# PaddlePaddle/Parakeet

Measured on AMD Instinct MI355X. Metric: audio samples/sec, FastSpeech2+PWGAN 22.05kHz, higher is better.
Workload: dtype f32 (3-term split-fp16 MFMA, fp32-equivalent; exact-fp32 in roofline.exact_f32); 1 GPU; FastSpeech2+PWG end-to-end (BASELINE config 4 per-GPU share): 32 utterances/GPU x 128 phonemes -> 640 frames -> 163840 samples each, LJSpeech architecture, random-init weights; utterances_per_gpu=32, global_batch=32, minibatch=32, parallelism=dp1 (utterance sharding, no data-path collective)

## Files before the change

parakeet_amd/csrc/pwg.hip:

```cpp
#include <cmath>
#include <cstdlib>

#include "pk_gemm.h"
#include "pk_split.h"
#include "pwg_gen.h"

typedef float f32x16 __attribute__((ext_vector_type(16)));
typedef float f32x4 __attribute__((ext_vector_type(4)));
typedef float f32x2 __attribute__((ext_vector_type(2)));
#ifndef PK_PWG_TILE_MAP
#define PK_PWG_TILE_MAP 1
#endif
#ifndef PK_PWG_NT_SKIP
#define PK_PWG_NT_SKIP 1
#endif
#ifndef PK_PWG_SKIP_SCOPE
#define PK_PWG_SKIP_SCOPE 0
#endif
#ifndef PK_PWG_NT_EDGE
#define PK_PWG_NT_EDGE 0
#endif
#ifndef PK_PWG_AMAX_PROBE
#define PK_PWG_AMAX_PROBE 0
#endif
#ifndef PK_PWG_NT_XOUT
#define PK_PWG_NT_XOUT 1
#endif
#ifndef PK_PWG_SKIP_VEC
#define PK_PWG_SKIP_VEC 1
#endif
#if PK_PWG_SKIP_VEC && PK_PWG_SKIP_SCOPE != 0
#error "PK_PWG_SKIP_SCOPE measures the dword skip stream: build it with PK_PWG_SKIP_VEC=0"
#endif
namespace {
__device__ __forceinline__ f32x4 pwg_skip_ld4(const float* p) {
#if PK_PWG_NT_SKIP
    return __builtin_nontemporal_load(reinterpret_cast<const f32x4*>(p));
#else
    return *reinterpret_cast<const f32x4*>(p);
#endif
}
__device__ __forceinline__ void pwg_skip_st4(f32x4 v, float* p) {
#if PK_PWG_NT_SKIP
    __builtin_nontemporal_store(v, reinterpret_cast<f32x4*>(p));
#else
    *reinterpret_cast<f32x4*>(p) = v;
#endif
}
__device__ __forceinline__ float pwg_skip_ld(const float* p) {
#if PK_PWG_SKIP_SCOPE == 1
    return __hip_atomic_load(p, __ATOMIC_RELAXED, __HIP_MEMORY_SCOPE_AGENT);
#elif PK_PWG_SKIP_SCOPE == 2
    return __hip_atomic_load(p, __ATOMIC_RELAXED, __HIP_MEMORY_SCOPE_SYSTEM);
#elif PK_PWG_SKIP_SCOPE == 3
    return __hip_atomic_load(p, __ATOMIC_RELAXED, __HIP_MEMORY_SCOPE_WORKGROUP);
#elif PK_PWG_NT_SKIP
    return __builtin_nontemporal_load(p);
#else
    return *p;
#endif
}
__device__ __forceinline__ void pwg_skip_st(float v, float* p) {
// ... 245 lines not shown
    float acc = 0.f;
    for (int jj = 0; jj < UPW; ++jj) acc = fmaf(w[jj], P[(long)(row0 + f + jj - 2) * ldp + col0 + co], acc);
    out[(long)co * n_frames * hop + (long)f * hop + phase] = acc;
}

struct PwgLayerArgs {
    const float* xin;
    float* xout;
    float* skip;
    const float* w1;
    const float* w2;
    const float* bias;
    const float* P;
    const float* uptab;
    const int* tile_t0;
    const int* tile_cls;
    long Ttot;
    int ldp;
    int ntiles;
    int dilation;
    int dbg;
    const unsigned* xe_in;
    unsigned* xe_out;
    int k1;
    float i0, i1;
    const int* tile_kx_in;
    const int* tile_kx_out;
    const float* noise;
    const float* nz_tab;
    float nz_wmax, nz_bmax;
    long noise_n;
    unsigned* amax_out;
    PwgGen gen;
};

__device__ __forceinline__ float gated(float a, float b) {
    a = __builtin_amdgcn_fmed3f(a, -10.f, 10.f);
    const float ea = __expf(-2.f * a);
    const float eb = __expf(-b);
    return (1.f - ea) * __builtin_amdgcn_rcpf((1.f + ea) * (1.f + eb));
}

constexpr float PK_Z_SCALE = PK_UNIT_SCALE;
template <int CTRL, int ROW_MASK>
__device__ __forceinline__ float dpp_max_step(float v) {
    const int t = __builtin_amdgcn_update_dpp(__float_as_int(v), __float_as_int(v), CTRL, ROW_MASK, 0xf, false);
    return fmaxf(v, __int_as_float(t));
}
__device__ __forceinline__ float wave_max64(float v) {
    v = dpp_max_step<0xB1, 0xf>(v);
    v = dpp_max_step<0x4E, 0xf>(v);
    v = dpp_max_step<0x124, 0xf>(v);
    v = dpp_max_step<0x128, 0xf>(v);
    v = dpp_max_step<0x142, 0xa>(v);
    v = dpp_max_step<0x143, 0xc>(v);
    return __int_as_float(__builtin_amdgcn_readlane(__float_as_int(v), 63));
}
__device__ __forceinline__ float gated_s(float a, float b, float ca, float cb) {
    const float ta = __builtin_amdgcn_fmed3f(a * ca, -28.853900817779268f, 28.853900817779268f);
    const float ea = __builtin_amdgcn_exp2f(ta);
    const float eb = __builtin_amdgcn_exp2f(b * cb);
    return fmaf(ea, -PK_Z_SCALE, PK_Z_SCALE) * __builtin_amdgcn_rcpf((1.f + ea) * (1.f + eb));
}

__device__ __forceinline__ f32x2 gated_s2(f32x2 a, f32x2 b, float ca, float cb) {
    f32x2 ta = a * ca, tb = b * cb;
// ... 278 lines not shown
}
typedef __fp16 pkh2 __attribute__((ext_vector_type(2)));
template <>
__device__ __forceinline__ void split_x8<f16x8, _Float16, true>(const float (&v)[8], f16x8& hi, f16x8& lo) {
#pragma unroll
    for (int p = 0; p < 4; ++p) {
        const pkh2 h = __builtin_amdgcn_cvt_pkrtz(v[2 * p], v[2 * p + 1]);
        const unsigned hu = __builtin_bit_cast(unsigned, h);
        float l0, l1;
        asm("v_fma_mix_f32 %0, %1, -1.0, %2 op_sel:[0,0,0] op_sel_hi:[1,0,0]" : "=v"(l0) : "v"(hu), "v"(v[2 * p]));
        asm("v_fma_mix_f32 %0, %1, -1.0, %2 op_sel:[1,0,0] op_sel_hi:[1,0,0]" : "=v"(l1) : "v"(hu), "v"(v[2 * p + 1]));
        hi[2 * p] = (_Float16)h[0];
        hi[2 * p + 1] = (_Float16)h[1];
        lo[2 * p] = (_Float16)l0;
        lo[2 * p + 1] = (_Float16)l1;
    }
}

__device__ __forceinline__ void split_x8s(const float (&v)[8], float s, f16x8& hi, f16x8& lo) {
    float t[8];
#pragma unroll
    for (int p = 0; p < 4; ++p) {
        f32x2 u = {v[2 * p], v[2 * p + 1]};
        u *= s;
        t[2 * p] = u[0];
        t[2 * p + 1] = u[1];
    }
    split_x8<f16x8, _Float16, true>(t, hi, lo);
}

template <bool FIRST, bool HALF, int ABL = 0, bool GEN = false, bool PL = false, bool AMAX = false, bool NZ = false>
__global__ __launch_bounds__(LAYER_WAVES * 64, LAYER_WAVES / 4) void k_pwg_layer_b3(PwgLayerArgs a) {
    static_assert(!NZ || (FIRST && PL && !GEN), "noise-fed: the first block of the planes path at hop 256");
    static_assert(!PL || (HALF && ABL == 0), "planes: the block-scaled split-fp16 path only");
    typedef typename Split16<HALF>::vec bf16x8;
    typedef typename Split16<HALF>::elem elem16;
    __shared__ __attribute__((aligned(16))) float lds[GEN ? LDS_TOTAL_GEN : LDS_TOTAL];
    float* lds_bias = lds + LDS_W1 + LDS_W2;
    {
        const f32x4* src = reinterpret_cast<const f32x4*>(NZ ? a.nz_tab : a.w1);
        f32x4* dst = reinterpret_cast<f32x4*>(lds);
        for (int i = threadIdx.x; i < (NZ ? (2048 + 128) * 4 : B3_W1_BYTES) / 16; i += LAYER_WAVES * 64) dst[i] = src[i];
        const f32x4* src2 = reinterpret_cast<const f32x4*>(a.w2);
        f32x4* dst2 = reinterpret_cast<f32x4*>(lds + LDS_W1);
        for (int i = threadIdx.x; i < B3_W2_BYTES / 16; i += LAYER_WAVES * 64) dst2[i] = src2[i];
        if (threadIdx.x < LDS_BIAS) lds_bias[threadIdx.x] = a.bias[threadIdx.x];
    }
    __syncthreads();

    const int lane = threadIdx.x & 63;
    const int wave = threadIdx.x >> 6;
    const int j = lane & 31;
    const int hi = lane >> 5;
    const int d = a.dilation;
    const bf16x8* lds_a = reinterpret_cast<const bf16x8*>(lds) + lane;
    const bf16x8* lds_a2 = reinterpret_cast<const bf16x8*>(lds + LDS_W1) + lane;
    float* lds_p = lds + LDS_W1 + LDS_W2 + LDS_BIAS + wave * (GEN ? LDS_PW_GEN : LDS_PW);

    const int per_xcd = gridDim.x >> 3;
    const int wg_slot = (gridDim.x & 7) == 0 ? (int)(blockIdx.x & 7) * per_xcd + (int)(blockIdx.x >> 3)
                                             : (int)blockIdx.x;
    int my_slot = wg_slot * LAYER_WAVES + wave;
#if PK_PWG_TILE_MAP
    static_assert(LAYER_WAVES == 8, "the tile maps below split a workgroup into waves 0..3 / 4..7 (wave >> 2, wave & 3) and the window into 8 per workgroup");
    if ((gridDim.x & 7) == 0) {
        const int wgl = (int)(blockIdx.x >> 3), win = per_xcd * LAYER_WAVES;
        const int local = PK_PWG_TILE_MAP == 1 ? (wave >> 2) * (win >> 1) + wgl * 4 + (wave & 3)
                        : PK_PWG_TILE_MAP == 2 ? wave * per_xcd + wgl
                                               : (wave & 3) * (win >> 2) + wgl * 2 + (wave >> 2);
        my_slot = (int)(blockIdx.x & 7) * win + local;
    }
#endif
    const int stride_slots = (int)gridDim.x * LAYER_WAVES;
    const int n_wtiles = a.ntiles * (TILE / WAVE_T);

    int eoff = 0;
    if (HALF) {
        const int dc = (d + 31) >> 5, df = d >> 5;
        eoff = lane == 0 ? -dc : (lane == 1 ? -df : (lane == 3 ? df : (lane == 4 ? dc : 0)));
    }
    auto load_amax = [&](int t0, int wt) -> unsigned {
        const long tt0 = (long)(t0 & ~255) + (wt & 7) * WAVE_T;
        return (ABL & 1) ? 0x3f800000u : a.xe_in[(tt0 >> 5) + eoff];
    };
    auto tile_scale_exp = [&](unsigned ev) -> int {
        unsigned m = (unsigned)__builtin_amdgcn_readlane((int)ev, 0);
        const unsigned m1 = (unsigned)__builtin_amdgcn_readlane((int)ev, 1);
        const unsigned m2 = (unsigned)__builtin_amdgcn_readlane((int)ev, 2);
        const unsigned m3 = (unsigned)__builtin_amdgcn_readlane((int)ev, 3);
        const unsigned m4 = (unsigned)__builtin_amdgcn_readlane((int)ev, 4);
        m = m > m1 ? m : m1;
        m = m > m2 ? m : m2;
        m = m > m3 ? m : m3;
        m = m > m4 ? m : m4;
        return blk_scale_exp(m);
    };
    int kx = 0, kx_next = 0;
    float xs_cur = 0.f;
    int kxn_v = 0;

    auto group_row = [&](int g, int e) -> long {
        const int cg = g / 3;
        return (long)(32 * (cg >> 1) + mfma_row(8 * (cg & 1) + e, 0));
    };
    auto lane_off = [&](int t0, int wt, int tap) -> unsigned {
        const long tt = (long)(t0 & ~255) + (wt & 7) * WAVE_T + j + (long)(tap - 1) * d;
        return (unsigned)(xoff(tt) + 4 * hi * XBLK);
// ... 39 lines not shown
            const PwgGenCoord gc = gen_coord(a.gen, tile, wt & 7, j);
            prow = a.gen.P0 + (long)(gc.row0 + gc.fa - 2) * a.ldp;
            wsel = (long)gc.cls * a.gen.hop + gc.phase;
            df_n = gc.df;
            valid_n = gc.valid;
        } else {
            prow = a.P + (long)(tile - 2) * a.ldp;
        }
#pragma unroll
        for (int it = 0; it < 3; ++it) {
            const int idx = lane + 64 * it;
            const int jj = idx >> 5, c4 = idx & 31;
            if (idx < (UPW + (GEN ? 1 : 0)) * (G / 4)) preg[it] = *reinterpret_cast<const f32x4*>(prow + (long)jj * a.ldp + 4 * c4);
        }
        if constexpr (!GEN) wsel = (long)cls * TILE + phase;
        const float* wrow = a.uptab + wsel * UPW_PAD;
        const f32x4 w0 = *reinterpret_cast<const f32x4*>(wrow);
        uw[0] = w0[0]; uw[1] = w0[1]; uw[2] = w0[2]; uw[3] = w0[3];
        uw[4] = wrow[4];
    };
    float nzn[3] = {0.f, 0.f, 0.f};
    int cls_cur = 0;
    auto nz_load = [&](int wt_) {
        const long i0 = (long)wt_ * WAVE_T + j;
#pragma unroll
        for (int k = 0; k < 3; ++k) {
            long i = i0 + k - 1;
            i = i < 0 ? 0 : (i >= a.noise_n ? a.noise_n - 1 : i);
            nzn[k] = a.noise[i];
        }
    };
    unsigned vo8n[3] = {0, 0, 0};
    unsigned pvo8n[3] = {0, 0, 0};
    if (my_slot < n_wtiles) {
        const int t0c = a.tile_t0[my_slot >> 3];
#pragma unroll
        for (int tp = 0; tp < 3; ++tp) {
            vo8n[tp] = lane_off(t0c, my_slot, tp);
            if constexpr (PL) pvo8n[tp] = lane_off_pl(t0c, my_slot, tp);
        }
        prefetch_head(my_slot, __builtin_amdgcn_readfirstlane(t0c & 255));
        if constexpr (NZ) {
            cls_cur = __builtin_amdgcn_readfirstlane(t0c & 255);
            kx = __builtin_amdgcn_readfirstlane(a.tile_kx_in[my_slot >> 3]);
            nz_load(my_slot);
        }
#pragma unroll
        for (int g = 0; g < (NZ ? 0 : B3_RING); ++g) load_group(ring[g], g, vo8n[g % 3], pvo8n[g % 3]);
        if constexpr (NZ) {
        } else if constexpr (PL) {
            kx = __builtin_amdgcn_readfirstlane(a.tile_kx_in[my_slot >> 3]);
            planes_operand(ring[0], ph, pl);
        } else if constexpr (HALF) {
            kx = tile_scale_exp(load_amax(t0c, my_slot));
            if constexpr ((ABL & 2) != 0) {
                ph = __builtin_bit_cast(bf16x8, f32x4{ring[0][0], ring[0][1], ring[0][2], ring[0][3]});
                pl = __builtin_bit_cast(bf16x8, f32x4{ring[0][4], ring[0][5], ring[0][6], ring[0][7]});
            } else
            split_x8s(ring[0], pow2f(kx), ph, pl);
        } else {
            split_x8<bf16x8, elem16, HALF>(ring[0], ph, pl);
        }
    }
    bf16x8 c_ah, c_al;
    if constexpr (!NZ) {
        c_ah = lds_a[0];
        c_al = lds_a[4 * 64];
    }

    int amax_utt = -1;
    unsigned amax_run = 0u;
    for (int wt = my_slot; wt < n_wtiles; wt += stride_slots) {
        const int next_wt = wt + stride_slots < n_wtiles ? wt + stride_slots : wt;
        unsigned vo8[3], pvo8[3];
#pragma unroll
        for (int tp = 0; tp < 3; ++tp) {
            vo8[tp] = vo8n[tp];
            pvo8[tp] = pvo8n[tp];
        }
        const int t0n = a.tile_t0[next_wt >> 3];
        int ko_v = 0;
        int utt_v = 0;
        if constexpr (PL) {
            kxn_v = a.tile_kx_in[next_wt >> 3];
            ko_v = a.tile_kx_out[wt >> 3];
            if constexpr (AMAX) utt_v = a.gen.tile_utt[wt >> 3];
            xs_cur = __uint_as_float(0x3f3504f3u - ((unsigned)kx << 23));
        }
        int cls_next = 0;
        const unsigned vo4 = vo8[1];
#if PK_PWG_SKIP_VEC
        const unsigned svo = (vo4 & ~(unsigned)(XBLK_FLOATS - 1)) + (unsigned)(128 * hi + 4 * j);
#endif
        float x_old[32];
        float nz_cur[3] = {0.f, 0.f, 0.f};
        if constexpr (NZ) {
#pragma unroll
            for (int k = 0; k < 3; ++k) nz_cur[k] = nzn[k];
            nz_load(next_wt);
        }
#pragma unroll
        for (int it = 0; it < 3; ++it) {
            const int idx = lane + 64 * it;
            if (idx < (UPW + (GEN ? 1 : 0)) * (G / 4)) reinterpret_cast<f32x4*>(lds_p)[idx] = preg[it];
        }
        const bool lane_valid = valid_n;
// ... 294 lines not shown
                        if (u != amax_utt) {
                            if (amax_utt >= 0 && lane == 0 && !PK_PWG_AMAX_PROBE)
                                atomicMax(a.amax_out + amax_utt * PWG_AMAX_PARTS + (int)(blockIdx.x & (PWG_AMAX_PARTS - 1)), amax_run);
                            amax_utt = u;
                            amax_run = m;
                        } else {
                            amax_run = amax_run > m ? amax_run : m;
                        }
                    }
                    if constexpr (PL) {
                        const float so = pow2f(__builtin_amdgcn_readfirstlane(ko_v));
                        char* pd = reinterpret_cast<char*>(a.xout) + pvo8[1];
#pragma unroll
                        for (int cg = 0; cg < 4; ++cg) {
                            float t8[8];
#pragma unroll
                            for (int e = 0; e < 8; ++e) t8[e] = acc2[cg >> 1][8 * (cg & 1) + e];
                            pl_f16x8 oh, ol;
                            split_x8s(t8, so, oh, ol);
                            if (PK_PWG_NT_XOUT) {
                                __builtin_nontemporal_store(oh, reinterpret_cast<pl_f16x8*>(pd + cg * 2048));
                                __builtin_nontemporal_store(ol, reinterpret_cast<pl_f16x8*>(pd + cg * 2048 + 16));
                            } else {
                                *reinterpret_cast<pl_f16x8*>(pd + cg * 2048) = oh;
                                *reinterpret_cast<pl_f16x8*>(pd + cg * 2048 + 16) = ol;
                            }
                        }
                    }
                }
            }
        }
        kx = kx_next;
        if constexpr (NZ) cls_cur = cls_next;
    }
    if constexpr (PL && AMAX) {
        if (amax_utt >= 0 && lane == 0 && !PK_PWG_AMAX_PROBE)
            atomicMax(a.amax_out + amax_utt * PWG_AMAX_PARTS + (int)(blockIdx.x & (PWG_AMAX_PARTS - 1)), amax_run);
    }
}

struct PwgLastArgs {
    const float* skip;
    const float* w1;
    const float* b1;
    const float* w2;
    float b2;
    float scale;
    const int* tile_t0;
    long Ttot;
    float* wav;
    int kw;
    PwgGen gen;
};
template <bool GEN>
__device__ __forceinline__ long last_out_index(const PwgLastArgs& a, int tile, int off, bool& valid) {
    if constexpr (GEN) {
        const int b = a.gen.tile_utt[tile];
        const int sidx = a.gen.tile_s0[tile] + off;
        valid = sidx < a.gen.utt_S[b];
        return (long)a.gen.utt_off[b] + sidx;
    } else {
        valid = true;
        return (long)tile * TILE + off;
    }
}

template <bool GEN>
__global__ __launch_bounds__(512) void k_pwg_last(PwgLastArgs a) {
    const int lane = threadIdx.x & 63;
    const int wave = threadIdx.x >> 6;
// ... 118 lines not shown
    bool finalized = false;
    int hop = 256;
    int max_dilation = 512;
    int gap = 512;
    bool use_norm = false;
    std::vector<float> h_mu, h_sigma;
    pk_dbuf d_first_w, d_first_b, d_convin_wT, d_uptab, d_mu, d_sigma;
    pk_dbuf d_w1, d_w2, d_bias;
    pk_dbuf d_w1b, d_w2b, d_w1h, d_w2h;
    int math = PK_PWG_MATH_F16X3;
    pk_dbuf d_waux;
    pk_dbuf d_l1, d_l1b, d_l2, d_l1h;
    float l2_bias = 0.f;
    std::vector<int> k1, k2o, k2s;
    int kw_last = 0;
    pk_dbuf d_bias_h, ws_xe0, ws_xe1;
    pk_dbuf ws_mel, ws_noise, ws_wav, ws_c0, ws_cin, ws_P, ws_x0, ws_x1, ws_skip, ws_dbg;
    pk_dbuf ws_tab;
    std::vector<int> last_frames, last_toff, last_cuL, last_cuC;
    float first_wmax = 0.f, first_bmax = 0.f;
    std::vector<float> first_w_host, first_b_host;
    pk_dbuf d_nz;
    int nz_k1 = 0;
    bool noise_fed = true;
    pk_dbuf d_cl, ws_nmax, ws_tkx;
    int last_ntiles = 0;
    long last_Ttot = 0;
    int last_x_final = 0;
    int last_ldp = 0;
    size_t last_o_cls = 0;
    int dbg = 0;
    bool planes_on = true;
    bool last_planes = false;
    bool last_skip_vec = false;
    int scale_guard = 1;
    bool guard_done = false;
    int guard_every = 16;
    int calls_since_sample = 0;
    int samples_dropped = 0;
    bool sample_pending = false;
    hipEvent_t ev_sample = nullptr;
    float* host_sample = nullptr;
    size_t host_sample_cap = 0;
    int sample_B = 0;
    std::vector<int> sample_frames;
    int deferred_fallbacks = 0;
    bool fell_back = false;
    std::vector<float> overshoot_log2;
    std::vector<float> cl_host;
    pk_dbuf ws_amax;
    unsigned long long seed = 0, rng_offset = 0;
    long chunk_samples = 1L << 40;
    bool generic_shape = false;
    bool generic_opt = false;
    bool gen_active = false;
    pwg_gen* gen = nullptr;
};

template <bool PROF>
static int pwg_ablation_launch(pk_ctx* ctx, int dbg, int grid, dim3 blk, const PwgLayerArgs& a) {
    if constexpr (PROF) {
        if (dbg == 1) PK_LAUNCH(ctx, "pwg_layer_h3", (k_pwg_layer_b3<false, true, 1>), dim3(grid), blk, 0, a);
        else if (dbg == 32) PK_LAUNCH(ctx, "pwg_layer_h3", (k_pwg_layer_b3<false, true, 2>), dim3(grid), blk, 0, a);
        else if (dbg == 96) PK_LAUNCH(ctx, "pwg_layer_h3", (k_pwg_layer_b3<false, true, 6>), dim3(grid), blk, 0, a);
        else if (dbg == 160) PK_LAUNCH(ctx, "pwg_layer_h3", (k_pwg_layer_b3<false, true, 10>), dim3(grid), blk, 0, a);
        else PK_LAUNCH(ctx, "pwg_layer_h3", (k_pwg_layer_b3<false, true>), dim3(grid), blk, 0, a);
        return PK_OK;
    } else {
        PK_FAIL(PK_ESTATE, "ablation switches exist in the profile build only");
    }
}

extern "C" int pk_pwg_create(pk_ctx* ctx, const pk_pwg_cfg* cfg, pk_pwg** out) {
    if (!ctx || !cfg || !out) PK_FAIL(PK_EINVAL, "pk_pwg_create: NULL argument");
    *out = nullptr;
    if (cfg->stacks <= 0 || cfg->layers <= 0 || cfg->layers % cfg->stacks != 0)
        PK_FAIL(PK_ESHAPE, "PWGGenerator: layers (%d) must be a positive multiple of stacks (%d)",
                cfg->layers, cfg->stacks);
    if (cfg->use_causal_conv) PK_FAIL(PK_EUNSUPPORTED, "PWGGenerator: use_causal_conv=True is not implemented");
    const bool generic_shape = cfg->in_channels != 1 || cfg->out_channels != 1 || cfg->kernel_size != KTAP ||
                               cfg->residual_channels != R || cfg->gate_channels != G || cfg->skip_channels != SK ||
                               cfg->aux_channels != AUX;
    if (generic_shape) PK_TRY(pwg_gen_check(*cfg));
    if (cfg->n_upsample < 1 || cfg->n_upsample > 8) PK_FAIL(PK_EINVAL, "PWGGenerator: 1..8 upsample scales");
    int hop = 1;
    double reach = 0.0;
    for (int i = 0; i < cfg->n_upsample; ++i) {
        int s = cfg->upsample_scales[i];
        if (s < 1 || 2 * s + 1 > MAX_UP_TAPS) PK_FAIL(PK_EUNSUPPORTED, "upsample scale %d unsupported", s);
        hop *= s;
        reach += (double)s / hop;
    }
    if (hop < WAVE_T || hop > 1024)
        PK_FAIL(PK_EUNSUPPORTED, "prod(upsample_scales) = %d: hop sizes from %d to 1024 are supported", hop, WAVE_T);
    if (reach >= 2.0) PK_FAIL(PK_EUNSUPPORTED, "upsample scales reach %.2f frames (>= 2)", reach);
    if (cfg->aux_context_window < 0 || cfg->aux_context_window > 8)
        PK_FAIL(PK_EINVAL, "aux_context_window out of range");
    int lps = cfg->layers / cfg->stacks;
    if (lps > 12) PK_FAIL(PK_EUNSUPPORTED, "dilation 2^%d too large", lps - 1);
    pk_pwg* h = new pk_pwg();
    h->ctx = ctx;
    h->cfg = *cfg;
    h->hop = hop;
    h->max_dilation = 1 << (lps - 1);
    h->gap = ((h->max_dilation + TILE - 1) / TILE) * TILE;
// ... 75 lines not shown
        (void)hipGetLastError();
        return;
    }
    h->sample_pending = false;
    if (st != hipSuccess) {
        (void)hipGetLastError();
        ++h->samples_dropped;
        return;
    }
    const int layers = (int)h->cl_host.size(), B = h->sample_B;
    const float worst = pwg_guard_verdict(h, h->host_sample, h->host_sample + (size_t)(layers + 1) * B, B, h->sample_frames.data());
    if (worst > PWG_GUARD_MAX_LOG2 && h->planes_on) {
        h->planes_on = false;
        h->fell_back = true;
        ++h->deferred_fallbacks;
    }
}

extern "C" int pk_pwg_set_option(pk_pwg* h, const char* key, int64_t value) {
    if (!h || !key) PK_FAIL(PK_EINVAL, "pk_pwg_set_option: NULL argument");
    if (strcmp(key, "planes") == 0) {
        h->planes_on = value != 0;
        if (h->planes_on) h->fell_back = false;
    } else if (strcmp(key, "scale_guard") == 0) {
        if (value < 0 || value > 2) PK_FAIL(PK_EINVAL, "pk_pwg_set_option: scale_guard %lld (0, 1, 2)", (long long)value);
        h->scale_guard = (int)value;
    } else if (strcmp(key, "noise_fed_first") == 0) {
        if (value < 0 || value > 1) PK_FAIL(PK_EINVAL, "pk_pwg_set_option: noise_fed_first %lld (0, 1)", (long long)value);
        h->noise_fed = value != 0;
    } else if (strcmp(key, "generic_kernel") == 0) {
        if (value < 0 || value > 1) PK_FAIL(PK_EINVAL, "pk_pwg_set_option: generic_kernel %lld (0, 1)", (long long)value);
        h->generic_opt = value != 0;
        h->finalized = false;
    } else if (strcmp(key, "scale_guard_every") == 0) {
        if (value < 0 || value > (1 << 30)) PK_FAIL(PK_EINVAL, "pk_pwg_set_option: scale_guard_every %lld", (long long)value);
        h->guard_every = (int)value;
    } else PK_FAIL(PK_EINVAL, "pk_pwg_set_option: unknown option '%s'", key);
    return PK_OK;
}

extern "C" int pk_pwg_scale_overshoot(pk_pwg* h, float* log2_overshoot, int32_t n, int32_t* fell_back) {
    if (!h || !log2_overshoot) PK_FAIL(PK_EINVAL, "pk_pwg_scale_overshoot: NULL argument");
    if (h->gen_active) PK_FAIL(PK_ESTATE, "pk_pwg_scale_overshoot: the generic path has no scale guard");
    {
        pk_device_guard _dg(h->ctx->device);
        pwg_poll_sample(h, true);
    }
    if (h->overshoot_log2.empty()) PK_FAIL(PK_ESTATE, "pk_pwg_scale_overshoot: no guarded inference has run (option \"scale_guard\")");
    if (n != (int32_t)h->overshoot_log2.size())
        PK_FAIL(PK_ESHAPE, "pk_pwg_scale_overshoot: expected %d floats (layers + 1)", (int)h->overshoot_log2.size());
    memcpy(log2_overshoot, h->overshoot_log2.data(), (size_t)n * sizeof(float));
    if (fell_back) *fell_back = h->fell_back ? (h->deferred_fallbacks > 0 ? 2 : 1) : 0;
    return PK_OK;
}

extern "C" int pk_pwg_set_seed(pk_pwg* h, uint64_t seed) {
    if (!h) PK_FAIL(PK_EINVAL, "pk_pwg_set_seed: handle is NULL");
    h->seed = seed;
    h->rng_offset = 0;
    return PK_OK;
}

static inline uint16_t f32_to_bf16_rne(float f) {
    uint32_t u;
    memcpy(&u, &f, 4);
    if ((u & 0x7fffffffu) > 0x7f800000u) return 0x7fc0;
// ... 504 lines not shown
        PK_TRY(h->ws_cin.reserve((size_t)(rows_p_alloc + 2 * P_LEAD) * AUX * 4));
        float* cin = h->ws_cin.as<float>() + (size_t)P_LEAD * AUX;
        PK_LAUNCH(ctx, "pwg_convin_prep", k_pwg_convin_prep, dim3(rows_p_alloc), dim3(128), 0, d_mel,
                  h->d_mu.as<float>(), h->d_sigma.as<float>(), (h->use_norm && (flags & PK_APPLY_NORMALIZER)) ? 1 : 0, d_tab + o_psrc, rows_p, cin);
        {
            pk_gemm_args g;
            g.A = cin;
            g.lda = AUX;
            g.Wp = h->d_convin_wT.as<float>();
            g.C = c0;
            g.ldc = AUX;
            g.M = rows_p;
            g.N = AUX;
            g.Cin = AUX;
            g.taps = kin;
            g.pad = cw;
            g.out_rowmap = d_tab + o_pout;
            PK_TRY(pk_gemm_launch(ctx, "pwg_convin_gemm", g));
        }
        pk_gemm_args g;
        g.A = c0;
        g.lda = AUX;
        g.Wp = h->d_waux.as<float>();
        g.C = P;
        g.ldc = ldp;
        g.M = sumL;
        g.N = ldp;
        g.Cin = AUX;
        g.taps = 1;
        g.pad = 0;
        PK_TRY(pk_gemm_launch(ctx, "pwg_aux_gemm", g));
    }
    const bool all_first = PK_PROFILE_BUILD != 0 && h->dbg == 1024;
    bool planes = h->planes_on && h->math == PK_PWG_MATH_F16X3 && (h->dbg == 0 || all_first) && (size_t)R * Ttot * 4 < ((size_t)1 << 32);
    constexpr float GUARD_MAX_LOG2 = PWG_GUARD_MAX_LOG2;
    const bool guard = planes && (h->scale_guard == 2 || (h->scale_guard == 1 && !h->guard_done));
    bool sample = false;
    if (planes && !guard && h->scale_guard == 1 && h->guard_every > 0 && !h->sample_pending &&
        ++h->calls_since_sample >= h->guard_every) {
        if (B <= PWG_SAMPLE_MAX_B && h->host_sample && h->ev_sample) sample = true;
        else ++h->samples_dropped;
        h->calls_since_sample = 0;
    }
    unsigned* amax = nullptr;
    if (guard || sample) {
        const size_t n_amax = (size_t)(c.layers + 1) * B + (size_t)c.layers * B * PWG_AMAX_PARTS;
        PK_TRY(h->ws_amax.reserve(n_amax * sizeof(unsigned)));
        amax = h->ws_amax.as<unsigned>();
        PK_HIP(hipMemsetAsync(amax, 0, n_amax * sizeof(unsigned), ctx->stream));
    }
    for (int attempt = 0;; ++attempt) {
    bool amax_parts_used = false;
    h->last_planes = planes;
    h->last_skip_vec = PK_PWG_SKIP_VEC != 0 && h->math != PK_PWG_MATH_F32;
    int* tkx = nullptr;
    if (planes) {
        PK_TRY(h->ws_nmax.reserve((size_t)B * 4));
        PK_TRY(h->ws_tkx.reserve((size_t)(c.layers + 1) * sumC * 4));
        tkx = h->ws_tkx.as<int>();
        PK_HIP(hipMemsetAsync(h->ws_nmax.p, 0, (size_t)B * 4, ctx->stream));
        PK_LAUNCH(ctx, "pwg_noise_max", k_pwg_noise_max, dim3(B, NMAX_PARTS), dim3(256), 0, d_noise, d_tab + o_uoff, d_tab + o_uS,
                  h->ws_nmax.as<float>());
        PK_LAUNCH(ctx, "pwg_tile_scales", k_pwg_tile_scales, dim3(pk_div_up(sumC, 256)), dim3(256), 0, d_tab + o_tutt, sumC,
                  h->ws_nmax.as<float>(), h->first_wmax, h->first_bmax, h->d_cl.as<float>(), c.layers, tkx);
    }
    const bool nz = planes && !gen && !all_first && h->noise_fed && h->d_nz.p != nullptr;
    if (nz) {
    } else if (planes && gen)
        PK_LAUNCH(ctx, "pwg_first", (k_pwg_first<true, true>), dim3(sumC), dim3(TILE), 0, d_noise, h->d_first_w.as<float>(),
                  h->d_first_b.as<float>(), d_tab + o_tile, Ttot, h->ws_x0.as<float>(), h->ws_xe0.as<unsigned>(), gtab, tkx);
    else if (planes)
        PK_LAUNCH(ctx, "pwg_first", (k_pwg_first<false, true>), dim3(sumC), dim3(TILE), 0, d_noise, h->d_first_w.as<float>(),
                  h->d_first_b.as<float>(), d_tab + o_tile, Ttot, h->ws_x0.as<float>(), h->ws_xe0.as<unsigned>(), gtab, tkx);
    else if (gen)
        PK_LAUNCH(ctx, "pwg_first", k_pwg_first<true>, dim3(sumC), dim3(TILE), 0, d_noise, h->d_first_w.as<float>(),
                  h->d_first_b.as<float>(), d_tab + o_tile, Ttot, h->ws_x0.as<float>(), h->ws_xe0.as<unsigned>(), gtab, tkx);
    else
        PK_LAUNCH(ctx, "pwg_first", k_pwg_first<false>, dim3(sumC), dim3(TILE), 0, d_noise, h->d_first_w.as<float>(),
                  h->d_first_b.as<float>(), d_tab + o_tile, Ttot, h->ws_x0.as<float>(), h->ws_xe0.as<unsigned>(), gtab, tkx);
    if (guard && planes && !nz)
        PK_LAUNCH(ctx, "pwg_planes_amax", k_pwg_planes_amax, dim3(sumC), dim3(256), 0, h->ws_x0.as<float>(), d_tab + o_tile,
                  d_tab + o_tutt, tkx, amax);
    {
        const int lps = c.layers / c.stacks;
        const int grid = ctx->n_cu;
        std::vector<int> chunk_first;
        {
            long acc = 0;
            for (int b = 0; b < B; ++b) {
                const long s_b = (long)frames[b] * hop;
                if (b == 0 || acc + s_b > h->chunk_samples) {
                    chunk_first.push_back(b);
                    acc = 0;
                }
                acc += s_b;
            }
            chunk_first.push_back(B);
        }
        for (size_t ck = 0; ck + 1 < chunk_first.size(); ++ck) {
        const int tile0 = cuC[chunk_first[ck]], ntile = cuC[chunk_first[ck + 1]] - tile0;
        const int row0 = cuL[chunk_first[ck]];
        for (int l = 0; l < c.layers; ++l) {
            PwgLayerArgs a;
            a.amax_out = nullptr;
            a.noise = nullptr;
            a.nz_tab = nullptr;
            a.noise_n = 0;
            a.nz_wmax = a.nz_bmax = 0.f;
            a.xin = (l & 1) ? h->ws_x1.as<float>() : h->ws_x0.as<float>();
            a.xout = (l & 1) ? h->ws_x0.as<float>() : h->ws_x1.as<float>();
            a.skip = h->ws_skip.as<float>();
            a.w1 = h->d_w1.as<float>() + (size_t)l * KS1 * 64 * 4;
            a.w2 = h->d_w2.as<float>() + (size_t)l * KS2 * 64 * 4;
            a.bias = h->d_bias.as<float>() + (size_t)l * (G + R + SK);
            a.P = P + (size_t)l * G + (size_t)row0 * ldp;
            a.gen = gtab;
            a.gen.tile_s0 += tile0;
            a.gen.tile_utt += tile0;
            a.gen.P0 = P + (size_t)l * G;
            a.uptab = h->d_uptab.as<float>();
            a.tile_t0 = d_tab + o_tile + tile0;
            a.tile_cls = d_tab + o_cls + tile0;
            a.Ttot = Ttot;
            a.ldp = ldp;
            a.ntiles = ntile;
            a.dilation = 1 << (l % lps);
            a.dbg = h->dbg;
            a.xe_in = (l & 1) ? h->ws_xe1.as<unsigned>() : h->ws_xe0.as<unsigned>();
            a.xe_out = (l & 1) ? h->ws_xe0.as<unsigned>() : h->ws_xe1.as<unsigned>();
            a.k1 = 0;
            a.i0 = a.i1 = 1.f;
            a.tile_kx_in = planes ? tkx + (size_t)l * sumC + tile0 : nullptr;
            a.tile_kx_out = planes ? tkx + (size_t)(l + 1) * sumC + tile0 : nullptr;
            if (h->math == PK_PWG_MATH_BF16X3 || h->math == PK_PWG_MATH_F16X3) {
                const bool half = h->math == PK_PWG_MATH_F16X3;
                if (half) {
                    a.bias = h->d_bias_h.as<float>() + (size_t)l * (G + R + SK);
                    a.k1 = h->k1[l];
                    a.i0 = (float)std::ldexp(0.70710678118654752440, -(14 + h->k2o[l]));
                    a.i1 = (float)std::ldexp(1.0, -(14 + h->k2s[l]));
                }
                a.w1 = reinterpret_cast<const float*>((half ? h->d_w1h : h->d_w1b).as<char>() + (size_t)l * B3_W1_BYTES);
                a.w2 = reinterpret_cast<const float*>((half ? h->d_w2h : h->d_w2b).as<char>() + (size_t)l * B3_W2_BYTES);
                const dim3 blk(LAYER_WAVES * 64);
                if (nz && l == 0) {
                    a.noise = d_noise + (size_t)tile0 * TILE;
                    a.noise_n = (long)sumS - (long)tile0 * TILE;
                    a.nz_tab = h->d_nz.as<float>();
                    a.nz_wmax = h->first_wmax;
                    a.nz_bmax = h->first_bmax;
                    a.k1 = h->nz_k1;
                }
                if (planes && (guard || sample) && !all_first) {
                    a.amax_out = amax + (size_t)(c.layers + 1) * B + (size_t)l * B * PWG_AMAX_PARTS;
                    amax_parts_used = true;
                    if (nz && l == 0) {
                        PK_LAUNCH(ctx, "pwg_layer_h3", (k_pwg_layer_b3<true, true, 0, false, true, true, true>), dim3(grid), blk, 0, a);
                    } else if (gen) {
                        if (l == 0) PK_LAUNCH(ctx, "pwg_layer_h3", (k_pwg_layer_b3<true, true, 0, true, true, true>), dim3(grid), blk, 0, a);
                        else PK_LAUNCH(ctx, "pwg_layer_h3", (k_pwg_layer_b3<false, true, 0, true, true, true>), dim3(grid), blk, 0, a);
                    } else {
                        if (l == 0) PK_LAUNCH(ctx, "pwg_layer_h3", (k_pwg_layer_b3<true, true, 0, false, true, true>), dim3(grid), blk, 0, a);
                        else PK_LAUNCH(ctx, "pwg_layer_h3", (k_pwg_layer_b3<false, true, 0, false, true, true>), dim3(grid), blk, 0, a);
                    }
                } else if (planes) {
                    if (gen) {
                        if (l == 0) PK_LAUNCH(ctx, "pwg_layer_h3", (k_pwg_layer_b3<true, true, 0, true, true>), dim3(grid), blk, 0, a);
                        else PK_LAUNCH(ctx, "pwg_layer_h3", (k_pwg_layer_b3<false, true, 0, true, true>), dim3(grid), blk, 0, a);
                    } else if (nz && l == 0) {
                        PK_LAUNCH(ctx, "pwg_layer_h3", (k_pwg_layer_b3<true, true, 0, false, true, false, true>), dim3(grid), blk, 0, a);
                    } else {
                        if (l == 0 || all_first) PK_LAUNCH(ctx, "pwg_layer_h3", (k_pwg_layer_b3<true, true, 0, false, true>), dim3(grid), blk, 0, a);
                        else PK_LAUNCH(ctx, "pwg_layer_h3", (k_pwg_layer_b3<false, true, 0, false, true>), dim3(grid), blk, 0, a);
                    }
                } else if (gen) {
                    if (half) {
                        if (l == 0) PK_LAUNCH(ctx, "pwg_layer_h3", (k_pwg_layer_b3<true, true, 0, true>), dim3(grid), blk, 0, a);
                        else PK_LAUNCH(ctx, "pwg_layer_h3", (k_pwg_layer_b3<false, true, 0, true>), dim3(grid), blk, 0, a);
                    } else {
                        if (l == 0) PK_LAUNCH(ctx, "pwg_layer_b3", (k_pwg_layer_b3<true, false, 0, true>), dim3(grid), blk, 0, a);
                        else PK_LAUNCH(ctx, "pwg_layer_b3", (k_pwg_layer_b3<false, false, 0, true>), dim3(grid), blk, 0, a);
                    }
                } else if (half) {
                    if (l == 0) PK_LAUNCH(ctx, "pwg_layer_h3", (k_pwg_layer_b3<true, true>), dim3(grid), blk, 0, a);
                    else if (h->dbg != 0) PK_TRY(pwg_ablation_launch<PK_PROFILE_BUILD != 0>(ctx, h->dbg, grid, blk, a));
                    else PK_LAUNCH(ctx, "pwg_layer_h3", (k_pwg_layer_b3<false, true>), dim3(grid), blk, 0, a);
                } else {
                    if (l == 0) PK_LAUNCH(ctx, "pwg_layer_b3", (k_pwg_layer_b3<true, false>), dim3(grid), blk, 0, a);
                    else PK_LAUNCH(ctx, "pwg_layer_b3", (k_pwg_layer_b3<false, false>), dim3(grid), blk, 0, a);
                }
            } else if (gen) {
                if (l == 0) PK_LAUNCH(ctx, "pwg_layer", (k_pwg_layer<true, true>), dim3(grid), dim3(LAYER_WAVES * 64), 0, a);
                else PK_LAUNCH(ctx, "pwg_layer", (k_pwg_layer<false, true>), dim3(grid), dim3(LAYER_WAVES * 64), 0, a);
            } else if (l == 0)
                PK_LAUNCH(ctx, "pwg_layer", (k_pwg_layer<true, false>), dim3(grid), dim3(LAYER_WAVES * 64), 0, a);
            else
                PK_LAUNCH(ctx, "pwg_layer", (k_pwg_layer<false, false>), dim3(grid), dim3(LAYER_WAVES * 64), 0, a);
            if ((guard || sample) && planes && all_first)
                PK_LAUNCH(ctx, "pwg_planes_amax", k_pwg_planes_amax, dim3(ntile), dim3(256), 0, a.xout, a.tile_t0, a.gen.tile_utt,
                          a.tile_kx_out, amax + (size_t)(l + 1) * B);
        }
        }
        h->last_x_final = c.layers & 1;
        if (amax_parts_used)
            PK_LAUNCH(ctx, "pwg_amax_fold", k_pwg_amax_fold, dim3(pk_div_up(c.layers * B, 256)), dim3(256), 0,
                      amax + (size_t)(c.layers + 1) * B, amax + B, c.layers * B);
    }
    if (sample) {
        const size_t n_am = (size_t)(c.layers + 1) * B;
        PK_HIP(hipMemcpyAsync(h->host_sample, amax, n_am * sizeof(float), hipMemcpyDeviceToHost, ctx->stream));
        PK_HIP(hipMemcpyAsync(h->host_sample + n_am, h->ws_nmax.p, (size_t)B * sizeof(float), hipMemcpyDeviceToHost, ctx->stream));
        PK_HIP(hipEventRecord(h->ev_sample, ctx->stream));
        h->sample_B = B;
        h->sample_frames.assign(frames, frames + B);
        h->sample_pending = true;
    }
    if (!(guard && attempt == 0)) break;
    {
        std::vector<float> am((size_t)(c.layers + 1) * B), nmax(B);
        PK_HIP(hipStreamSynchronize(ctx->stream));
        PK_HIP(hipMemcpy(am.data(), amax, am.size() * sizeof(float), hipMemcpyDeviceToHost));
        PK_HIP(hipMemcpy(nmax.data(), h->ws_nmax.p, (size_t)B * sizeof(float), hipMemcpyDeviceToHost));
        const float worst = pwg_guard_verdict(h, am.data(), nmax.data(), B, frames);
        h->guard_done = true;
        if (worst <= GUARD_MAX_LOG2) break;
        h->planes_on = false;
        h->fell_back = true;
        planes = false;
    }
    }
    {
        PwgLastArgs a;
        a.skip = h->ws_skip.as<float>();
        a.w1 = h->d_l1.as<float>();
        a.b1 = h->d_l1b.as<float>();
        a.w2 = h->d_l2.as<float>();
// ... 79 lines not shown
        return PK_OK;
    }
    if (what == 2 && h->last_skip_vec) {
        const long nblk = (S + XBLK - 1) / XBLK, blk0 = h->last_toff[b] / XBLK;
        std::vector<float> raw((size_t)nblk * XBLK_FLOATS);
        PK_HIP(hipMemcpy(raw.data(), src + (size_t)blk0 * XBLK_FLOATS, raw.size() * sizeof(float), hipMemcpyDeviceToHost));
        for (long bi = 0; bi < nblk; ++bi)
            for (int ch = 0; ch < SK; ++ch)
                for (int sidx = 0; sidx < XBLK && bi * XBLK + sidx < S; ++sidx)
                    host_out[(size_t)ch * S + bi * XBLK + sidx] = raw[(size_t)bi * XBLK_FLOATS + (size_t)(ch >> 2) * (4 * XBLK) + sidx * 4 + (ch & 3)];
        return PK_OK;
    }
    for (int ch = 0; ch < rows; ++ch) {
        if (S / XBLK > 0)
            PK_HIP(hipMemcpy2D(host_out + (size_t)ch * S, XBLK * sizeof(float),
                               src + xoff(h->last_toff[b]) + (size_t)ch * XBLK, XBLK_FLOATS * sizeof(float),
                               XBLK * sizeof(float), S / XBLK, hipMemcpyDeviceToHost));
        if (S % XBLK)
            PK_HIP(hipMemcpy(host_out + (size_t)ch * S + S / XBLK * XBLK,
                             src + xoff(h->last_toff[b] + S / XBLK * XBLK) + (size_t)ch * XBLK,
                             (size_t)(S % XBLK) * sizeof(float), hipMemcpyDeviceToHost));
    }
    return PK_OK;
}

extern "C" void pk_pwg_destroy(pk_pwg* h) {
    if (!h) return;
    pk_device_guard _dg(h->ctx->device);
    (void)hipStreamSynchronize(h->ctx->stream);
    pk_dbuf* bufs[] = {&h->d_first_w, &h->d_first_b, &h->d_convin_wT, &h->d_uptab, &h->d_mu, &h->d_sigma,
                       &h->d_w1, &h->d_w2, &h->d_bias, &h->d_w1b, &h->d_w2b, &h->d_w1h, &h->d_w2h, &h->d_waux, &h->d_nz, &h->d_l1, &h->d_l1h, &h->d_l1b, &h->d_l2,
                       &h->d_bias_h, &h->ws_xe0, &h->ws_xe1,
                       &h->ws_mel, &h->ws_cin, &h->ws_noise, &h->ws_wav, &h->ws_c0, &h->ws_P,
                       &h->ws_x0, &h->ws_x1, &h->ws_skip, &h->ws_dbg, &h->ws_tab, &h->d_cl, &h->ws_nmax, &h->ws_tkx, &h->ws_amax};
    for (auto* b : bufs) b->release();
    if (h->host_sample) (void)hipHostFree(h->host_sample);
    if (h->ev_sample) (void)hipEventDestroy(h->ev_sample);
    pwg_gen_destroy(h->gen);
    delete h;
}
```

Before: 123.6 million samples/s.

## Add intra-workgroup tile stealing and a global tail pool to PWG layer kernel

```diff
diff --git a/parakeet_amd/csrc/pwg.hip b/parakeet_amd/csrc/pwg.hip
--- a/parakeet_amd/csrc/pwg.hip
+++ b/parakeet_amd/csrc/pwg.hip
@@ -28,6 +28,15 @@
 #endif
 #ifndef PK_PWG_SKIP_VEC
 #define PK_PWG_SKIP_VEC 1
+#endif
+#ifndef PK_PWG_TILE_SHARE
+#define PK_PWG_TILE_SHARE 1
+#endif
+#ifndef PK_PWG_TILE_POOL
+#define PK_PWG_TILE_POOL 3
+#endif
+#ifndef PK_PWG_TILE_SHARE_MIN_SWEEPS
+#define PK_PWG_TILE_SHARE_MIN_SWEEPS 12
 #endif
 #if PK_PWG_SKIP_VEC && PK_PWG_SKIP_SCOPE != 0
 #error "PK_PWG_SKIP_SCOPE measures the dword skip stream: build it with PK_PWG_SKIP_VEC=0"
@@ -339,6 +348,10 @@
     long noise_n;
     unsigned* amax_out;
     PwgGen gen;
+    int tile_share;
+    unsigned* pool;
+    int pool_first;
+    unsigned long long* stamps;
 };
 
 __device__ __forceinline__ float gated(float a, float b) {
@@ -683,11 +696,26 @@
 template <bool FIRST, bool HALF, int ABL = 0, bool GEN = false, bool PL = false, bool AMAX = false, bool NZ = false>
 __global__ __launch_bounds__(LAYER_WAVES * 64, LAYER_WAVES / 4) void k_pwg_layer_b3(PwgLayerArgs a) {
     static_assert(!NZ || (FIRST && PL && !GEN), "noise-fed: the first block of the planes path at hop 256");
-    static_assert(!PL || (HALF && ABL == 0), "planes: the block-scaled split-fp16 path only");
+    static_assert(!PL || (HALF && (ABL == 0 || ABL == 16)), "planes: the block-scaled split-fp16 path only (ablations: the wave stamps)");
     typedef typename Split16<HALF>::vec bf16x8;
     typedef typename Split16<HALF>::elem elem16;
     __shared__ __attribute__((aligned(16))) float lds[GEN ? LDS_TOTAL_GEN : LDS_TOTAL];
+    __shared__ unsigned share_cnt[2 * LAYER_WAVES];
     float* lds_bias = lds + LDS_W1 + LDS_W2;
+    auto stamp = [&](int i) {
+        if constexpr ((ABL & 16) != 0) {
+            if ((threadIdx.x & 63) == 0) {
+                unsigned long long* r = a.stamps + ((size_t)blockIdx.x * LAYER_WAVES + (threadIdx.x >> 6)) * 8;
+                r[2 * i] = __builtin_amdgcn_s_memrealtime();
+                r[2 * i + 1] = __builtin_amdgcn_s_memtime();
+            }
+        }
+    };
+    stamp(0);
+    if (threadIdx.x == 0) {
+#pragma unroll
+        for (int v = 0; v < 2 * LAYER_WAVES; ++v) share_cnt[v] = 0u;
+    }
     {
         const f32x4* src = reinterpret_cast<const f32x4*>(NZ ? a.nz_tab : a.w1);
         f32x4* dst = reinterpret_cast<f32x4*>(lds);
@@ -698,6 +726,7 @@
         if (threadIdx.x < LDS_BIAS) lds_bias[threadIdx.x] = a.bias[threadIdx.x];
     }
     __syncthreads();
+    stamp(1);
 
     const int lane = threadIdx.x & 63;
     const int wave = threadIdx.x >> 6;
@@ -711,19 +740,53 @@
     const int per_xcd = gridDim.x >> 3;
     const int wg_slot = (gridDim.x & 7) == 0 ? (int)(blockIdx.x & 7) * per_xcd + (int)(blockIdx.x >> 3)
                                              : (int)blockIdx.x;
-    int my_slot = wg_slot * LAYER_WAVES + wave;
+    static_assert(LAYER_WAVES == 8, "the tile maps below split a workgroup into waves 0..3 / 4..7 (wave >> 2, wave & 3) and the window into 8 per workgroup");
+    auto slot_of = [&](int w) -> int {
 #if PK_PWG_TILE_MAP
-    static_assert(LAYER_WAVES == 8, "the tile maps below split a workgroup into waves 0..3 / 4..7 (wave >> 2, wave & 3) and the window into 8 per workgroup");
-    if ((gridDim.x & 7) == 0) {
-        const int wgl = (int)(blockIdx.x >> 3), win = per_xcd * LAYER_WAVES;
-        const int local = PK_PWG_TILE_MAP == 1 ? (wave >> 2) * (win >> 1) + wgl * 4 + (wave & 3)
-                        : PK_PWG_TILE_MAP == 2 ? wave * per_xcd + wgl
-                                               : (wave & 3) * (win >> 2) + wgl * 2 + (wave >> 2);
-        my_slot = (int)(blockIdx.x & 7) * win + local;
-    }
+        if ((gridDim.x & 7) == 0) {
+            const int wgl = (int)(blockIdx.x >> 3), win = per_xcd * LAYER_WAVES;
+            const int local = PK_PWG_TILE_MAP == 1 ? (w >> 2) * (win >> 1) + wgl * 4 + (w & 3)
+                            : PK_PWG_TILE_MAP == 2 ? w * per_xcd + wgl
+                                                   : (w & 3) * (win >> 2) + wgl * 2 + (w >> 2);
+            return (int)(blockIdx.x & 7) * win + local;
+        }
 #endif
+        return wg_slot * LAYER_WAVES + w;
+    };
+    const int my_slot = slot_of(wave);
     const int stride_slots = (int)gridDim.x * LAYER_WAVES;
     const int n_wtiles = a.ntiles * (TILE / WAVE_T);
+    const int n_list = a.pool ? (a.pool_first < n_wtiles ? a.pool_first : n_wtiles) : n_wtiles;
+    const int wave_u = __builtin_amdgcn_readfirstlane(wave);
+    const int share = a.tile_share;
+    int vic = (share == 2 && wave_u < 4) || (share == 3 && wave_u >= 4) ? 1 : 0;
+    auto grab = [&]() -> int {
+        while (vic < LAYER_WAVES) {
+            const int v = wave_u ^ ((vic >> 1) | ((vic & 1) << 2));
+            const int s = slot_of(v);
+            const int len = s < n_list ? (n_list - s + stride_slots - 1) / stride_slots : 0;
+            if (len > 0) {
+                const unsigned inc = vic == 0 ? 1u : 1u << 16;
+                unsigned r = 0u;
+                if (lane == 0) r = atomicAdd(&share_cnt[v], inc) + inc;
+                r = (unsigned)__builtin_amdgcn_readlane((int)r, 0);
+                const int front = (int)(r & 0xffffu), back = (int)(r >> 16);
+                if (front + back <= len) return s + (vic == 0 ? front - 1 : len - back) * stride_slots;
+            }
+            ++vic;
+        }
+        if (vic == LAYER_WAVES) {
+            if (a.pool) {
+                unsigned r = 0u;
+                if (lane == 0) r = atomicAdd(a.pool, 1u);
+                r = (unsigned)__builtin_amdgcn_readlane((int)r, 0);
+                if (r < (unsigned)(n_wtiles - n_list)) return n_list + (int)r;
+            }
+            vic = LAYER_WAVES + 1;
+        }
+        return -1;
+    };
+    const int first_wt = __builtin_amdgcn_readfirstlane(share ? grab() : (my_slot < n_wtiles ? my_slot : -1));
 
     int eoff = 0;
     if (HALF) {
@@ -829,27 +892,27 @@
     };
     unsigned vo8n[3] = {0, 0, 0};
     unsigned pvo8n[3] = {0, 0, 0};
-    if (my_slot < n_wtiles) {
-        const int t0c = a.tile_t0[my_slot >> 3];
+    if (first_wt >= 0) {
+        const int t0c = a.tile_t0[first_wt >> 3];
 #pragma unroll
         for (int tp = 0; tp < 3; ++tp) {
-            vo8n[tp] = lane_off(t0c, my_slot, tp);
-            if constexpr (PL) pvo8n[tp] = lane_off_pl(t0c, my_slot, tp);
-        }
-        prefetch_head(my_slot, __builtin_amdgcn_readfirstlane(t0c & 255));
+            vo8n[tp] = lane_off(t0c, first_wt, tp);
+            if constexpr (PL) pvo8n[tp] = lane_off_pl(t0c, first_wt, tp);
+        }
+        prefetch_head(first_wt, __builtin_amdgcn_readfirstlane(t0c & 255));
         if constexpr (NZ) {
             cls_cur = __builtin_amdgcn_readfirstlane(t0c & 255);
-            kx = __builtin_amdgcn_readfirstlane(a.tile_kx_in[my_slot >> 3]);
-            nz_load(my_slot);
+            kx = __builtin_amdgcn_readfirstlane(a.tile_kx_in[first_wt >> 3]);
+            nz_load(first_wt);
         }
 #pragma unroll
         for (int g = 0; g < (NZ ? 0 : B3_RING); ++g) load_group(ring[g], g, vo8n[g % 3], pvo8n[g % 3]);
         if constexpr (NZ) {
         } else if constexpr (PL) {
-            kx = __builtin_amdgcn_readfirstlane(a.tile_kx_in[my_slot >> 3]);
+            kx = __builtin_amdgcn_readfirstlane(a.tile_kx_in[first_wt >> 3]);
             planes_operand(ring[0], ph, pl);
         } else if constexpr (HALF) {
-            kx = tile_scale_exp(load_amax(t0c, my_slot));
+            kx = tile_scale_exp(load_amax(t0c, first_wt));
             if constexpr ((ABL & 2) != 0) {
                 ph = __builtin_bit_cast(bf16x8, f32x4{ring[0][0], ring[0][1], ring[0][2], ring[0][3]});
                 pl = __builtin_bit_cast(bf16x8, f32x4{ring[0][4], ring[0][5], ring[0][6], ring[0][7]});
@@ -867,8 +930,18 @@
 
     int amax_utt = -1;
     unsigned amax_run = 0u;
-    for (int wt = my_slot; wt < n_wtiles; wt += stride_slots) {
-        const int next_wt = wt + stride_slots < n_wtiles ? wt + stride_slots : wt;
+    for (int wt = first_wt; wt >= 0;) {
+        int next_wt;
+        if (share) {
+            const int g = grab();
+            next_wt = g >= 0 ? g : wt;
+        } else {
+            next_wt = wt + stride_slots < n_wtiles ? wt + stride_slots : wt;
+        }
+        next_wt = __builtin_amdgcn_readfirstlane(next_wt);
+        if constexpr ((ABL & 16) != 0) {
+            if (lane == 0) atomicAdd(&share_cnt[LAYER_WAVES + wave], 1u);
+        }
         unsigned vo8[3], pvo8[3];
 #pragma unroll
         for (int tp = 0; tp < 3; ++tp) {
@@ -1229,10 +1302,20 @@
         }
         kx = kx_next;
         if constexpr (NZ) cls_cur = cls_next;
+        if (next_wt == wt) break;
+        wt = next_wt;
     }
     if constexpr (PL && AMAX) {
         if (amax_utt >= 0 && lane == 0 && !PK_PWG_AMAX_PROBE)
             atomicMax(a.amax_out + amax_utt * PWG_AMAX_PARTS + (int)(blockIdx.x & (PWG_AMAX_PARTS - 1)), amax_run);
+    }
+    stamp(2);
+    if constexpr ((ABL & 16) != 0) {
+        if (lane == 0) {
+            unsigned long long* r = a.stamps + ((size_t)blockIdx.x * LAYER_WAVES + wave) * 8;
+            r[6] = share_cnt[LAYER_WAVES + wave];
+            r[7] = (unsigned long long)blockIdx.x | (unsigned long long)wave << 32 | (unsigned long long)(__builtin_amdgcn_s_getreg(20 | (3 << 11)) & 15u) << 48;
+        }
     }
 }
 
@@ -1417,6 +1500,10 @@
     int dbg = 0;
     bool planes_on = true;
     bool last_planes = false;
+    int tile_share = PK_PWG_TILE_SHARE;
+    bool tile_share_set = false;
+    int tile_pool = -1;
+    pk_dbuf ws_stamps;
     bool last_skip_vec = false;
     int scale_guard = 1;
     bool guard_done = false;
@@ -1456,6 +1543,16 @@
     }
 }
 
+template <bool PROF>
+static int pwg_stamps_launch(pk_ctx* ctx, int grid, dim3 blk, const PwgLayerArgs& a) {
+    if constexpr (PROF) {
+        PK_LAUNCH(ctx, "pwg_layer_h3", (k_pwg_layer_b3<false, true, 16, false, true>), dim3(grid), blk, 0, a);
+        return PK_OK;
+    } else {
+        PK_FAIL(PK_ESTATE, "ablation switches exist in the profile build only");
+    }
+}
+
 extern "C" int pk_pwg_create(pk_ctx* ctx, const pk_pwg_cfg* cfg, pk_pwg** out) {
     if (!ctx || !cfg || !out) PK_FAIL(PK_EINVAL, "pk_pwg_create: NULL argument");
     *out = nullptr;
@@ -1597,6 +1694,13 @@
         if (value < 0 || value > 1) PK_FAIL(PK_EINVAL, "pk_pwg_set_option: generic_kernel %lld (0, 1)", (long long)value);
         h->generic_opt = value != 0;
         h->finalized = false;
+    } else if (strcmp(key, "tile_share") == 0) {
+        if (value < 0 || value > 3) PK_FAIL(PK_EINVAL, "pk_pwg_set_option: tile_share %lld (0, 1; 2, 3 = test modes)", (long long)value);
+        h->tile_share = (int)value;
+        h->tile_share_set = true;
+    } else if (strcmp(key, "tile_pool") == 0) {
+        if (value < -1 || value > 4096) PK_FAIL(PK_EINVAL, "pk_pwg_set_option: tile_pool %lld (-1 = default, 0 .. 4096 sweeps)", (long long)value);
+        h->tile_pool = (int)value;
     } else if (strcmp(key, "scale_guard_every") == 0) {
         if (value < 0 || value > (1 << 30)) PK_FAIL(PK_EINVAL, "pk_pwg_set_option: scale_guard_every %lld", (long long)value);
         h->guard_every = (int)value;
@@ -2167,7 +2271,8 @@
         PK_TRY(pk_gemm_launch(ctx, "pwg_aux_gemm", g));
     }
     const bool all_first = PK_PROFILE_BUILD != 0 && h->dbg == 1024;
-    bool planes = h->planes_on && h->math == PK_PWG_MATH_F16X3 && (h->dbg == 0 || all_first) && (size_t)R * Ttot * 4 < ((size_t)1 << 32);
+    const bool stamps = PK_PROFILE_BUILD != 0 && h->dbg == 256;
+    bool planes = h->planes_on && h->math == PK_PWG_MATH_F16X3 && (h->dbg == 0 || all_first || stamps) && (size_t)R * Ttot * 4 < ((size_t)1 << 32);
     constexpr float GUARD_MAX_LOG2 = PWG_GUARD_MAX_LOG2;
     const bool guard = planes && (h->scale_guard == 2 || (h->scale_guard == 1 && !h->guard_done));
     bool sample = false;
@@ -2190,10 +2295,10 @@
     h->last_skip_vec = PK_PWG_SKIP_VEC != 0 && h->math != PK_PWG_MATH_F32;
     int* tkx = nullptr;
     if (planes) {
-        PK_TRY(h->ws_nmax.reserve((size_t)B * 4));
+        PK_TRY(h->ws_nmax.reserve((size_t)(B + B * c.layers) * 4));
         PK_TRY(h->ws_tkx.reserve((size_t)(c.layers + 1) * sumC * 4));
         tkx = h->ws_tkx.as<int>();
-        PK_HIP(hipMemsetAsync(h->ws_nmax.p, 0, (size_t)B * 4, ctx->stream));
+        PK_HIP(hipMemsetAsync(h->ws_nmax.p, 0, (size_t)(B + B * c.layers) * 4, ctx->stream));
         PK_LAUNCH(ctx, "pwg_noise_max", k_pwg_noise_max, dim3(B, NMAX_PARTS), dim3(256), 0, d_noise, d_tab + o_uoff, d_tab + o_uS,
                   h->ws_nmax.as<float>());
         PK_LAUNCH(ctx, "pwg_tile_scales", k_pwg_tile_scales, dim3(pk_div_up(sumC, 256)), dim3(256), 0, d_tab + o_tutt, sumC,
@@ -2219,6 +2324,11 @@
     {
         const int lps = c.layers / c.stacks;
         const int grid = ctx->n_cu;
+        const size_t stamp_words = (size_t)grid * LAYER_WAVES * 8;
+        if (stamps) {
+            PK_TRY(h->ws_stamps.reserve((size_t)c.layers * stamp_words * sizeof(unsigned long long)));
+            PK_HIP(hipMemsetAsync(h->ws_stamps.p, 0, (size_t)c.layers * stamp_words * sizeof(unsigned long long), ctx->stream));
+        }
         std::vector<int> chunk_first;
         {
             long acc = 0;
@@ -2235,6 +2345,8 @@
         for (size_t ck = 0; ck + 1 < chunk_first.size(); ++ck) {
         const int tile0 = cuC[chunk_first[ck]], ntile = cuC[chunk_first[ck + 1]] - tile0;
         const int row0 = cuL[chunk_first[ck]];
+        if (h->tile_share != 0 && h->math != PK_PWG_MATH_F32 && (ntile + grid - 1) / grid + LAYER_WAVES >= 65536)
+            PK_FAIL(PK_EUNSUPPORTED, "pk_pwg_infer: %d tiles on %d workgroups are beyond the 16-bit list counters of option tile_share; set it to 0", ntile, grid);
         for (int l = 0; l < c.layers; ++l) {
             PwgLayerArgs a;
             a.amax_out = nullptr;
@@ -2261,6 +2373,18 @@
             a.ntiles = ntile;
             a.dilation = 1 << (l % lps);
             a.dbg = h->dbg;
+            const int sweeps = (ntile + grid - 1) / grid;
+            a.tile_share = h->tile_share_set || sweeps >= PK_PWG_TILE_SHARE_MIN_SWEEPS ? h->tile_share : 0;
+            a.pool = nullptr;
+            a.pool_first = 0;
+            if (planes && a.tile_share != 0) {
+                const int pool_sweeps = h->tile_pool >= 0 ? h->tile_pool : (sweeps >= PK_PWG_TILE_SHARE_MIN_SWEEPS ? PK_PWG_TILE_POOL : 0);
+                if (pool_sweeps > 0) {
+                    a.pool = h->ws_nmax.as<unsigned>() + B + ck * c.layers + l;
+                    a.pool_first = std::max(0, sweeps - pool_sweeps) * grid * LAYER_WAVES;
+                }
+            }
+            a.stamps = stamps ? h->ws_stamps.as<unsigned long long>() + (size_t)l * stamp_words : nullptr;
             a.xe_in = (l & 1) ? h->ws_xe1.as<unsigned>() : h->ws_xe0.as<unsigned>();
             a.xe_out = (l & 1) ? h->ws_xe0.as<unsigned>() : h->ws_xe1.as<unsigned>();
             a.k1 = 0;
@@ -2304,6 +2428,8 @@
                         else PK_LAUNCH(ctx, "pwg_layer_h3", (k_pwg_layer_b3<false, true, 0, true, true>), dim3(grid), blk, 0, a);
                     } else if (nz && l == 0) {
                         PK_LAUNCH(ctx, "pwg_layer_h3", (k_pwg_layer_b3<true, true, 0, false, true, false, true>), dim3(grid), blk, 0, a);
+                    } else if (stamps && l > 0) {
+                        PK_TRY(pwg_stamps_launch<PK_PROFILE_BUILD != 0>(ctx, grid, blk, a));
                     } else {
                         if (l == 0 || all_first) PK_LAUNCH(ctx, "pwg_layer_h3", (k_pwg_layer_b3<true, true, 0, false, true>), dim3(grid), blk, 0, a);
                         else PK_LAUNCH(ctx, "pwg_layer_h3", (k_pwg_layer_b3<false, true, 0, false, true>), dim3(grid), blk, 0, a);
@@ -2337,6 +2463,16 @@
         }
         }
         h->last_x_final = c.layers & 1;
+        if (stamps) {
+            if (const char* path = pk_prof_env("PK_PWG_STAMPS_OUT")) {
+                std::vector<unsigned long long> st((size_t)c.layers * stamp_words);
+                PK_HIP(hipStreamSynchronize(ctx->stream));
+                PK_HIP(hipMemcpy(st.data(), h->ws_stamps.p, st.size() * sizeof(unsigned long long), hipMemcpyDeviceToHost));
+                FILE* f = fopen(path, "wb");
+                if (!f || fwrite(st.data(), sizeof(unsigned long long), st.size(), f) != st.size()) PK_FAIL(PK_EINVAL, "PK_PWG_STAMPS_OUT: cannot write '%s'", path);
+                fclose(f);
+            }
+        }
         if (amax_parts_used)
             PK_LAUNCH(ctx, "pwg_amax_fold", k_pwg_amax_fold, dim3(pk_div_up(c.layers * B, 256)), dim3(256), 0,
                       amax + (size_t)(c.layers + 1) * B, amax + B, c.layers * B);
@@ -2482,7 +2618,7 @@
                        &h->d_w1, &h->d_w2, &h->d_bias, &h->d_w1b, &h->d_w2b, &h->d_w1h, &h->d_w2h, &h->d_waux, &h->d_nz, &h->d_l1, &h->d_l1h, &h->d_l1b, &h->d_l2,
                        &h->d_bias_h, &h->ws_xe0, &h->ws_xe1,
                        &h->ws_mel, &h->ws_cin, &h->ws_noise, &h->ws_wav, &h->ws_c0, &h->ws_P,
-                       &h->ws_x0, &h->ws_x1, &h->ws_skip, &h->ws_dbg, &h->ws_tab, &h->d_cl, &h->ws_nmax, &h->ws_tkx, &h->ws_amax};
+                       &h->ws_x0, &h->ws_x1, &h->ws_skip, &h->ws_dbg, &h->ws_tab, &h->d_cl, &h->ws_nmax, &h->ws_tkx, &h->ws_amax, &h->ws_stamps};
     for (auto* b : bufs) b->release();
     if (h->host_sample) (void)hipHostFree(h->host_sample);
     if (h->ev_sample) (void)hipEventDestroy(h->ev_sample);
```

New measurement: 124.6 million samples/s (median of 6 runs). Within noise of the previous version (+0.8%).
